# NthPortal/reservoir

Measured on AMD Instinct MI355X. Metric: elements sampled/sec (Gelem/s) + % HBM roofline, 1B Long keys k=1024, 1/2/4/8 GPU, higher is better.
Workload: dtype int64

## Files before the change

### reservoir_amd/csrc/rsv_elements.hip

```cpp
#include <algorithm>

#include "rsv_device.h"
#include "rsv_internal.h"
#include "rsv_scan.h"

namespace rsv {

namespace {

constexpr int kBlock = 256;

constexpr int kK1Unroll = 2;

constexpr unsigned kK1Grid = 256 * 20;

constexpr int kK1Win = 12;
struct K1Lds {
    uint64_t q[kBlock / 64][k1q_cap<kK1Win>()];
    uint64_t cq[kBlock / 64][kQueue];
};

__global__ __launch_bounds__(kBlock) void k1_last_writer(DrawKey dk, uint32_t k, uint64_t lo,
                                                         uint64_t hi, uint64_t g_begin,
                                                         uint64_t n_groups,
                                                         unsigned long long* __restrict__ win, K1Launch P) {
    __shared__ K1Lds L;
    const int w = threadIdx.x >> 6;
    if (P.flags & kK1Fast) k1_body_q<kK1Win, true, kBlock>(dk, k, lo, hi, g_begin, n_groups, win, L.q[w], L.cq[w], P);
    else k1_body_q<kK1Win, false, kBlock>(dk, k, lo, hi, g_begin, n_groups, win, L.q[w], L.cq[w], P);
}

template <typename Take, typename Empty, typename Keep>
__device__ __forceinline__ void slot_rule(int64_t j, unsigned long long wi, int64_t base, int64_t n, int fresh,
                                          Take&& take, Empty&& empty, Keep&& keep) {
    if (wi) take((int64_t)wi - base, (int64_t)wi, true);
    else if (j >= base && j < base + n) take(j - base, j, false);
    else if (fresh) empty((int64_t)-1);
    else keep();
}

template <typename KeyT, int R, bool kAgentWin>
__device__ __forceinline__ void resolve_registers_first(const KeyT* __restrict__ keys, int64_t base, int64_t n,
                                                        uint32_t k, unsigned long long* __restrict__ win,
                                                        KeyT* __restrict__ slot_key, int64_t* __restrict__ slot_idx,
                                                        int fresh, int64_t m, KeyT* dst, uint32_t* flag, uint32_t gen) {
    unsigned long long wi[R];
    KeyT v[R];
#pragma unroll
    for (int r = 0; r < R; ++r) {
        const uint32_t j = threadIdx.x + r * kBlock;
        if (j >= k) wi[r] = 0ull;
        else if (kAgentWin) wi[r] = __hip_atomic_load(&win[j], __ATOMIC_RELAXED, __HIP_MEMORY_SCOPE_AGENT);
        else wi[r] = win[j];
    }
#pragma unroll
    for (int r = 0; r < R; ++r) {
        const int64_t j = threadIdx.x + r * kBlock;
        if (j >= k) continue;
        KeyT x;
        slot_rule(
            j, wi[r], base, n, fresh, [&](int64_t off, int64_t, bool) { x = keys[off]; }, [&](int64_t) { x = 0; },
            [&] { x = slot_key[j]; });
        v[r] = x;
    }
#pragma unroll
    for (int r = 0; r < R; ++r) {
        const int64_t j = threadIdx.x + r * kBlock;
        if (j >= k) continue;
        const KeyT x = v[r];
        slot_rule(
            j, wi[r], base, n, fresh,
            [=](int64_t, int64_t idx, bool winner) {
                slot_key[j] = x;
                slot_idx[j] = idx;
                if (winner) win[j] = 0;
            },
            [=](int64_t idx) {
                slot_key[j] = 0;
                slot_idx[j] = idx;
            },
            [] {});
        if (j < m) dst[j] = x;
    }
    publish_flag(flag, gen);
}

constexpr uint32_t kK1FusedMaxK = 8 * kBlock;

template <typename KeyT>
__global__ __launch_bounds__(kBlock) void k1_resolve_publish(DrawKey dk, uint32_t k, uint64_t lo, uint64_t hi,
                                                             uint64_t g_begin, uint64_t n_groups,
                                                             unsigned long long* __restrict__ win,
                                                             uint32_t* ticket, const KeyT* __restrict__ keys,
                                                             int64_t base, int64_t n, KeyT* __restrict__ slot_key,
                                                             int64_t* __restrict__ slot_idx, int fresh, int64_t m,
                                                             KeyT* dst, uint32_t* flag, uint32_t gen, K1Launch P) {
    __shared__ K1Lds L;
    __shared__ uint32_t last;
    const int w = threadIdx.x >> 6;
    if (P.flags & kK1Fast) k1_body_q<kK1Win, true, kBlock>(dk, k, lo, hi, g_begin, n_groups, win, L.q[w], L.cq[w], P);
    else k1_body_q<kK1Win, false, kBlock>(dk, k, lo, hi, g_begin, n_groups, win, L.q[w], L.cq[w], P);
    asm volatile("s_waitcnt vmcnt(0)" ::: "memory");
    __syncthreads();
    if (threadIdx.x == 0) {
        const uint32_t prev = __hip_atomic_fetch_add(ticket, 1u, __ATOMIC_RELAXED, __HIP_MEMORY_SCOPE_AGENT);
        last = prev == gridDim.x - 1;
        if (last) __hip_atomic_store(ticket, 0u, __ATOMIC_RELAXED, __HIP_MEMORY_SCOPE_AGENT);
    }
    __syncthreads();
    if (!last) return;
    __builtin_amdgcn_fence(__ATOMIC_ACQUIRE, "agent");
    resolve_registers_first<KeyT, kK1FusedMaxK / kBlock, true>(keys, base, n, k, win, slot_key, slot_idx, fresh, m, dst,
                                                               flag, gen);
}

template <typename KeyT, bool kPublish>
__global__ __launch_bounds__(kPublish ? 1024 : kBlock) void resolve_kernel(const KeyT* __restrict__ keys, int64_t base,
                                                                         int64_t n, uint32_t k,
                                                                         unsigned long long* __restrict__ win,
                                                                         KeyT* __restrict__ slot_key,
                                                                         int64_t* __restrict__ slot_idx, int fresh,
                                                                         int64_t m, KeyT* dst, uint32_t* flag,
                                                                         uint32_t gen) {
    const uint32_t stride = gridDim.x * blockDim.x;
    for (uint32_t j = blockIdx.x * blockDim.x + threadIdx.x; j < k; j += stride) {
        KeyT v = 0;
        slot_rule(
            j, win[j], base, n, fresh,
            [&](int64_t off, int64_t idx, bool winner) {
                slot_key[j] = v = keys[off];
                if (kPublish || slot_idx) slot_idx[j] = idx;
                if (winner) win[j] = 0;
            },
            [=](int64_t idx) {
                slot_key[j] = 0;
                if (kPublish || slot_idx) slot_idx[j] = idx;
            },
            [&] {
                if (kPublish) v = slot_key[j];
            });
        if (kPublish && (int64_t)j < m) dst[j] = v;
    }
    if (kPublish) publish_flag(flag, gen);
}

template <typename KeyT, int R>
__global__ __launch_bounds__(kBlock) void resolve_publish_small_kernel(const KeyT* __restrict__ keys, int64_t base,
                                                                       int64_t n, uint32_t k,
                                                                       unsigned long long* __restrict__ win,
                                                                       KeyT* __restrict__ slot_key,
                                                                       int64_t* __restrict__ slot_idx, int fresh,
                                                                       int64_t m, KeyT* dst, uint32_t* flag, uint32_t gen) {
    resolve_registers_first<KeyT, R, false>(keys, base, n, k, win, slot_key, slot_idx, fresh, m, dst, flag, gen);
}

__global__ __launch_bounds__(kBlock) void replay_kernel(const int64_t* __restrict__ ev_pos,
                                                        const int32_t* __restrict__ ev_slot,
                                                        int64_t n_events, uint32_t k,
                                                        unsigned long long* __restrict__ win) {
    const int64_t e = (int64_t)blockIdx.x * blockDim.x + threadIdx.x;
    if (e >= n_events) return;
    const int32_t s = ev_slot[e];
    const int64_t p = ev_pos[e];
    if (s >= 0 && (uint32_t)s < k && p >= 2) atomicMax(&win[s], (unsigned long long)(p - 1));
}

__global__ __launch_bounds__(kBlock) void export_draws_kernel(DrawKey dk, uint64_t i0, int64_t n,
                                                              uint64_t* __restrict__ out) {
    const int64_t t = (int64_t)blockIdx.x * blockDim.x + threadIdx.x;
    if (t >= n) return;
    const uint64_t i = i0 + (uint64_t)t;
    const u32x4 w = level0(dk, i >> 4);
    out[t] = exact_j(dk, i, level0_byte(w, (uint32_t)(i & 15)));
}

template <typename KeyT>
struct StridedParts {
    using Key = KeyT;
    const int64_t* idx;
    const KeyT* key;
    int64_t part_len;
    __device__ int64_t index(int32_t p, uint32_t j) const { return idx[(int64_t)p * part_len + j]; }
    __device__ void take(int32_t p, uint32_t j, KeyT* slot_key) const { slot_key[j] = key[(int64_t)p * part_len + j]; }
};

template <typename KeyT>
struct PackedRows {
    using Key = KeyT;
    const int64_t* rows;
    int64_t stride;
    uint32_t k;
    __device__ int64_t index(int32_t p, uint32_t j) const { return rows[(int64_t)p * stride + j]; }
    __device__ void take(int32_t p, uint32_t j, KeyT* slot_key) const {
        slot_key[j] = (KeyT)rows[(int64_t)p * stride + k + j];
    }
};

struct StridedWideParts {
    using Key = uint32_t;
    const int64_t* idx;
    const uint32_t* key;
    int64_t part_len;
    uint32_t words;
    __device__ int64_t index(int32_t p, uint32_t j) const { return idx[(int64_t)p * part_len + j]; }
    __device__ void take(int32_t p, uint32_t j, uint32_t* slot_key) const {
        const uint32_t* src = key + ((size_t)p * part_len + j) * words;
        for (uint32_t q = 0; q < words; ++q) slot_key[(size_t)j * words + q] = src[q];
    }
};

struct PackedWideRows {
    using Key = uint32_t;
    const int64_t* rows;
    int64_t stride;
    uint32_t k, words;
    __device__ int64_t index(int32_t p, uint32_t j) const { return rows[(int64_t)p * stride + j]; }
    __device__ void take(int32_t p, uint32_t j, uint32_t* slot_key) const {
        const uint32_t* src = (const uint32_t*)(rows + (int64_t)p * stride + k) + (size_t)j * words;
        for (uint32_t q = 0; q < words; ++q) slot_key[(size_t)j * words + q] = src[q];
    }
};

template <typename Src>
__device__ __forceinline__ int32_t merge_winner(const Src& src, int32_t parts, uint32_t j, int64_t& best) {
    int32_t from = -1;
    for (int32_t p = 0; p < parts; ++p) {
        const int64_t idx = src.index(p, j);
        if (idx > best) {
            best = idx;
            from = p;
        }
    }
    return from;
}

template <typename Src, bool kPublish>
__global__ __launch_bounds__(kPublish ? 1024 : kBlock) void merge_kernel(Src src, int32_t parts, uint32_t k,
                                                                       int64_t* __restrict__ slot_idx,
                                                                       typename Src::Key* __restrict__ slot_key,
                                                                       int64_t m, typename Src::Key* dst,
                                                                       uint32_t* flag, uint32_t gen) {
    const uint32_t stride = gridDim.x * blockDim.x;
    for (uint32_t j = blockIdx.x * blockDim.x + threadIdx.x; j < k; j += stride) {
        int64_t best = slot_idx[j];
        const int32_t from = merge_winner(src, parts, j, best);
        if (from >= 0) {
            slot_idx[j] = best;
            src.take(from, j, slot_key);
        }
        if (kPublish && (int64_t)j < m) dst[j] = slot_key[j];
    }
    if (kPublish) publish_flag(flag, gen);
}

template <typename KeyT>
__global__ __launch_bounds__(kBlock) void export_packed_kernel(const int64_t* __restrict__ slot_idx,
                                                               const KeyT* __restrict__ slot_key, uint32_t k,
                                                               int64_t* __restrict__ row) {
    const uint32_t j = blockIdx.x * blockDim.x + threadIdx.x;
    if (j >= k) return;
    row[j] = slot_idx[j];
    row[k + j] = (int64_t)slot_key[j];
}

__global__ __launch_bounds__(1024) void resolve_wide_kernel(const uint32_t* __restrict__ keys, int64_t base,
                                                            int64_t n, uint32_t k, uint32_t words,
                                                            unsigned long long* __restrict__ win,
                                                            uint32_t* __restrict__ slot_key,
                                                            int64_t* __restrict__ slot_idx, int fresh, int64_t m,
                                                            uint32_t* dst, uint32_t* flag, uint32_t gen) {
    const uint32_t stride = gridDim.x * blockDim.x;
    for (uint32_t j = blockIdx.x * blockDim.x + threadIdx.x; j < k; j += stride) {
        const uint32_t* src = nullptr;
        bool write = true;
        slot_rule(
            j, win[j], base, n, fresh,
            [&](int64_t off, int64_t idx, bool winner) {
                src = keys + (size_t)off * words;
                slot_idx[j] = idx;
                if (winner) win[j] = 0;
            },
            [=](int64_t idx) { slot_idx[j] = idx; }, [&] { write = false; });
        uint32_t* o = slot_key + (size_t)j * words;
        const bool out = dst && (int64_t)j < m;
        for (uint32_t q = 0; q < words; ++q) {
            const uint32_t v = src ? src[q] : (write ? 0u : o[q]);
            if (write) o[q] = v;
            if (out) dst[(size_t)j * words + q] = v;
        }
    }
    if (dst) publish_flag(flag, gen);
}

__global__ __launch_bounds__(kBlock) void export_packed_wide_kernel(const int64_t* __restrict__ slot_idx,
                                                                    const uint32_t* __restrict__ slot_key, uint32_t k,
                                                                    uint32_t words, int64_t* __restrict__ row) {
    const uint32_t j = blockIdx.x * blockDim.x + threadIdx.x;
    if (j >= k) return;
    row[j] = slot_idx[j];
    uint32_t* o = (uint32_t*)(row + k) + (size_t)j * words;
    for (uint32_t q = 0; q < words; ++q) o[q] = slot_key[(size_t)j * words + q];
}

inline DrawKey make_key(const DrawParams& dp) {
    return DrawKey{(uint32_t)dp.seed, (uint32_t)(dp.seed >> 32), (uint32_t)dp.stream,
                   (uint32_t)(dp.stream >> 32)};
}

inline unsigned grid_for(uint64_t items, unsigned cap = ~0u) {
    uint64_t b = (items + kBlock - 1) / kBlock;
    if (b < 1) b = 1;
    return (unsigned)(b < cap ? b : cap);
}

inline unsigned k1_grid(uint64_t n_groups) {
    constexpr uint64_t per_window = (uint64_t)kK1Unroll * kBlock * kK1Win;
    if (n_groups < per_window * 768) return grid_for((n_groups + kK1Unroll - 1) / kK1Unroll, kK1Grid);
    const uint64_t m = std::max<uint64_t>(1, (n_groups + per_window * kK1Grid / 2) / (per_window * kK1Grid));
    return (unsigned)std::max<uint64_t>(1, n_groups / (per_window * m));
}

constexpr uint32_t kK1W1 = 256 * 6 * (kBlock / 64);
constexpr uint32_t kK1Rest = 5400, kK1MinA = 5;
inline unsigned k1_plan(uint32_t k, uint64_t lo, uint64_t hi, uint64_t g_begin, uint64_t n_groups, K1Launch& P) {
    const unsigned stride_grid = k1_grid(n_groups);
    P = k1_launch<kK1Win>(k, lo, hi, g_begin, n_groups, stride_grid, kBlock);
    if (P.units < kK1MinA * kK1W1 + kK1Rest) return stride_grid;
    const unsigned grid = k1_schedule(P, kK1W1, (P.units - kK1Rest) / kK1W1, 2, kBlock);
    return grid ? grid : stride_grid;
}

template <typename F>
hipError_t with_key_type(int key_width, F&& f) {
    if (key_width == 8) f(int64_t{});
    else f(int32_t{});
    return hipGetLastError();
}

inline unsigned one_group_threads(uint32_t k) {
    return std::min<unsigned>(1024, std::max<unsigned>(64, (k + 63) / 64 * 64));
}

}

hipError_t launch_k1_last_writer(const DrawParams& dp, uint32_t k, uint64_t lo, uint64_t hi,
                                 unsigned long long* batch_win, hipStream_t st) {
    if (hi <= lo) return hipSuccess;
    const uint64_t g_end = (hi + 15) >> 4;
    constexpr uint64_t kMaxGroups = 1ull << 31;
    uint64_t n_groups = 0;
    for (uint64_t g_begin = lo >> 4; g_begin < g_end; g_begin += n_groups) {
        const uint64_t g_wrap = ((g_begin >> 32) + 1) << 32;
        n_groups = std::min<uint64_t>(std::min<uint64_t>(g_end, g_wrap) - g_begin, kMaxGroups);
        K1Launch P;
        const unsigned grid = k1_plan(k, lo, hi, g_begin, n_groups, P);
        hipLaunchKernelGGL(k1_last_writer, dim3(grid), dim3(kBlock), 0, st, make_key(dp), k, lo, hi,
                           g_begin, n_groups, batch_win, P);
        hipError_t e = hipGetLastError();
        if (e != hipSuccess) return e;
    }
    return hipSuccess;
}

bool k1_fused_ok(uint64_t lo, uint64_t hi, uint32_t k, int key_width) {
    if (hi <= lo || k > kK1FusedMaxK || (key_width != 8 && key_width != 4)) return false;
    const uint64_t g_begin = lo >> 4, g_end = (hi + 15) >> 4;
    return g_end - g_begin <= (1ull << 31) && g_end <= ((g_begin >> 32) + 1) << 32;
}

hipError_t launch_k1_resolve_publish(const DrawParams& dp, uint64_t lo, uint64_t hi, const SlotBlock& sb,
                                     uint32_t* ticket, const Batch& b, const Publication& pub, hipStream_t st) {
    if (!k1_fused_ok(lo, hi, sb.k, sb.key_width)) return hipErrorInvalidValue;
    const uint64_t g_begin = lo >> 4, n_groups = ((hi + 15) >> 4) - g_begin;
    K1Launch P;
    const unsigned grid = k1_plan(sb.k, lo, hi, g_begin, n_groups, P);
    return with_key_type(sb.key_width, [&](auto t) {
        using T = decltype(t);
        hipLaunchKernelGGL(k1_resolve_publish<T>, dim3(grid), dim3(kBlock), 0, st, make_key(dp), sb.k, lo, hi, g_begin,
                           n_groups, sb.win, ticket, (const T*)b.keys, b.base, b.n, (T*)sb.slot_key, sb.slot_idx,
                           (int)b.fresh, pub.m, (T*)pub.dst, pub.flag, pub.gen, P);
    });
}

hipError_t launch_resolve(const SlotBlock& sb, const Batch& b, const Publication& pub, hipStream_t st, bool small) {
    const uint32_t k = sb.k;
    if (sb.key_width > 8) {
        const unsigned grid = pub.dst ? 1 : grid_for(k, 256 * 64);
        hipLaunchKernelGGL(resolve_wide_kernel, dim3(grid), dim3(pub.dst ? one_group_threads(k) : kBlock), 0, st,
                           (const uint32_t*)b.keys, b.base, b.n, k, (uint32_t)sb.key_width / 4, sb.win,
                           (uint32_t*)sb.slot_key, sb.slot_idx, (int)b.fresh, pub.m, (uint32_t*)pub.dst, pub.flag,
                           pub.gen);
        return hipGetLastError();
    }
    return with_key_type(sb.key_width, [&](auto t) {
        using T = decltype(t);
        auto go = [&](auto kernel, unsigned grid, unsigned threads) {
            hipLaunchKernelGGL(kernel, dim3(grid), dim3(threads), 0, st, (const T*)b.keys, b.base, b.n, k, sb.win,
                               (T*)sb.slot_key, sb.slot_idx, (int)b.fresh, pub.m, (T*)pub.dst, pub.flag, pub.gen);
        };
        if (!pub.dst) go(resolve_kernel<T, false>, grid_for(k), kBlock);
        else if (!(small && k <= 8 * kBlock)) go(resolve_kernel<T, true>, 1, one_group_threads(k));
        else if (k <= 2 * kBlock) go(resolve_publish_small_kernel<T, 2>, 1, kBlock);
        else if (k <= 4 * kBlock) go(resolve_publish_small_kernel<T, 4>, 1, kBlock);
        else go(resolve_publish_small_kernel<T, 8>, 1, kBlock);
    });
}

__global__ __launch_bounds__(kBlock) void init_slots_kernel(uint8_t* slot_key, int key_width, int64_t* slot_idx,
                                                            unsigned long long* win, uint32_t k, uint32_t* ticket) {
    const uint64_t stride = (uint64_t)gridDim.x * blockDim.x;
    if (ticket && blockIdx.x == 0 && threadIdx.x == 0) *ticket = 0;
    for (uint64_t j = (uint64_t)blockIdx.x * blockDim.x + threadIdx.x; j < k; j += stride) {
        win[j] = 0;
        slot_idx[j] = -1;
        if (key_width == 8)
            ((int64_t*)slot_key)[j] = 0;
        else if (key_width == 4)
            ((int32_t*)slot_key)[j] = 0;
        else
            for (int q = 0; q < key_width / 4; ++q) ((uint32_t*)slot_key)[(size_t)j * (key_width / 4) + q] = 0;
    }
}

hipError_t launch_init_slots(const SlotBlock& sb, hipStream_t st, uint32_t* ticket) {
    hipLaunchKernelGGL(init_slots_kernel, dim3(grid_for(sb.k, 256 * 64)), dim3(kBlock), 0, st, (uint8_t*)sb.slot_key,
                       sb.key_width, sb.slot_idx, sb.win, sb.k, ticket);
    return hipGetLastError();
}

__global__ __launch_bounds__(1024) void publish_kernel(const uint32_t* __restrict__ src, uint32_t* dst,
                                                      int64_t words, uint32_t* flag, uint32_t gen) {
    const int64_t vecs = words >> 2;
    for (int64_t i = threadIdx.x; i < vecs; i += blockDim.x)
        ((uint4*)dst)[i] = ((const uint4*)src)[i];
    for (int64_t i = (vecs << 2) + threadIdx.x; i < words; i += blockDim.x) dst[i] = src[i];
    publish_flag(flag, gen);
}

__global__ __launch_bounds__(1024) void publish_multi_kernel(const uint32_t* __restrict__ src, uint32_t* dst,
                                                            int64_t words, uint32_t* flag, uint32_t gen,
                                                            uint32_t* ticket) {
    const int64_t vecs = words >> 2;
    const int64_t stride = (int64_t)gridDim.x * blockDim.x;
    const int64_t t0 = (int64_t)blockIdx.x * blockDim.x + threadIdx.x;
    for (int64_t i = t0; i < vecs; i += stride) ((uint4*)dst)[i] = ((const uint4*)src)[i];
    for (int64_t i = (vecs << 2) + t0; i < words; i += stride) dst[i] = src[i];
    asm volatile("s_waitcnt vmcnt(0)" ::: "memory");
    __syncthreads();
    if (threadIdx.x == 0) {
        __threadfence_system();
        const uint32_t prev = __hip_atomic_fetch_add(ticket, 1u, __ATOMIC_ACQ_REL, __HIP_MEMORY_SCOPE_AGENT);
        if (prev == gridDim.x - 1) {
            __hip_atomic_store(ticket, 0u, __ATOMIC_RELAXED, __HIP_MEMORY_SCOPE_AGENT);
            __threadfence_system();
            __hip_atomic_store(flag, gen, __ATOMIC_RELEASE, __HIP_MEMORY_SCOPE_SYSTEM);
        }
    }
}

hipError_t launch_publish_multi(const void* src, int64_t bytes, void* dst_host_dev, uint32_t* flag_dev, uint32_t gen,
                                uint32_t* ticket_dev, hipStream_t st) {
    const int64_t per = 32 * 1024;
    const unsigned grid = (unsigned)std::min<int64_t>(32, std::max<int64_t>(1, (bytes + per - 1) / per));
    hipLaunchKernelGGL(publish_multi_kernel, dim3(grid), dim3(1024), 0, st, (const uint32_t*)src,
                       (uint32_t*)dst_host_dev, bytes / 4, flag_dev, gen, ticket_dev);
    return hipGetLastError();
}

hipError_t launch_publish(const void* src, int64_t bytes, void* dst_host_dev, uint32_t* flag_dev, uint32_t gen,
                          hipStream_t st) {
    hipLaunchKernelGGL(publish_kernel, dim3(1), dim3(1024), 0, st, (const uint32_t*)src, (uint32_t*)dst_host_dev,
                       bytes / 4, flag_dev, gen);
    return hipGetLastError();
}

__device__ __forceinline__ int64_t resolve_index_slot(uint64_t j, int64_t base, int64_t n, unsigned long long* win,
                                                      int64_t* slot_idx, int fresh, uint8_t* slot_key, int key_width) {
    int64_t off = -1;
    slot_rule(
        (int64_t)j, win[j], base, n, fresh,
        [&](int64_t o, int64_t idx, bool winner) {
            slot_idx[j] = idx;
            if (winner) win[j] = 0;
            off = o;
        },
        [=](int64_t idx) {
            slot_idx[j] = idx;
            for (int q = 0; q < key_width; ++q) slot_key[j * key_width + q] = 0;
        },
        [] {});
    return off;
}

__global__ __launch_bounds__(kBlock) void resolve_indices_kernel(int64_t base, int64_t n, uint32_t k,
                                                                 unsigned long long* __restrict__ win,
                                                                 int64_t* __restrict__ slot_idx, int fresh,
                                                                 uint8_t* __restrict__ slot_key, int key_width,
                                                                 int64_t* __restrict__ offs) {
    const uint64_t stride = (uint64_t)gridDim.x * blockDim.x;
    for (uint64_t j = (uint64_t)blockIdx.x * blockDim.x + threadIdx.x; j < k; j += stride)
        offs[j] = resolve_index_slot(j, base, n, win, slot_idx, fresh, slot_key, key_width);
}

__global__ __launch_bounds__(kBlock) void fill_slots_kernel(const int64_t* __restrict__ offs, const uint8_t* __restrict__ keys,
                                                            uint32_t k, int key_width, uint8_t* __restrict__ slot_key) {
    const uint64_t stride = (uint64_t)gridDim.x * blockDim.x;
    for (uint64_t j = (uint64_t)blockIdx.x * blockDim.x + threadIdx.x; j < k; j += stride) {
        if (offs[j] < 0) continue;
        if (key_width == 8) ((int64_t*)slot_key)[j] = ((const int64_t*)keys)[j];
        else if (key_width == 4) ((int32_t*)slot_key)[j] = ((const int32_t*)keys)[j];
        else
            for (int q = 0; q < key_width; ++q) slot_key[j * key_width + q] = keys[j * key_width + q];
    }
}


constexpr uint32_t kIdxPublishMaxK = 8192;

__global__ __launch_bounds__(1024) void resolve_indices_publish_kernel(int64_t base, int64_t n, uint32_t k,
                                                                       unsigned long long* __restrict__ win,
                                                                       int64_t* __restrict__ slot_idx, int fresh,
                                                                       uint8_t* __restrict__ slot_key, int key_width,
                                                                       int64_t* __restrict__ offs, int64_t* offs_host,
                                                                       uint32_t* flag, uint32_t gen) {
    for (uint32_t j = threadIdx.x; j < k; j += blockDim.x) {
        const int64_t off = resolve_index_slot(j, base, n, win, slot_idx, fresh, slot_key, key_width);
        offs[j] = off;
        offs_host[j] = off;
    }
    publish_flag(flag, gen);
}

template <typename KeyT>
__global__ __launch_bounds__(1024) void fill_slots_publish_kernel(const int64_t* __restrict__ offs,
                                                                  const KeyT* __restrict__ keys, uint32_t k,
                                                                  KeyT* __restrict__ slot_key, int64_t m, KeyT* dst,
                                                                  uint32_t* flag, uint32_t gen) {
    for (uint32_t j = threadIdx.x; j < k; j += blockDim.x) {
        KeyT v;
        if (offs[j] >= 0) {
            v = keys[j];
            slot_key[j] = v;
        } else {
            v = slot_key[j];
        }
        if ((int64_t)j < m) dst[j] = v;
    }
    publish_flag(flag, gen);
}

bool resolve_indices_publish_ok(uint32_t k) { return k <= kIdxPublishMaxK; }

hipError_t launch_resolve_indices(const SlotBlock& sb, const Batch& b, int64_t* offs, const Publication& pub,
                                  hipStream_t st) {
    if (!pub.dst)
        hipLaunchKernelGGL(resolve_indices_kernel, dim3(grid_for(sb.k, 256 * 64)), dim3(kBlock), 0, st, b.base, b.n, sb.k,
                           sb.win, sb.slot_idx, (int)b.fresh, (uint8_t*)sb.slot_key, sb.key_width, offs);
    else if (!resolve_indices_publish_ok(sb.k))
        return hipErrorInvalidValue;
    else
        hipLaunchKernelGGL(resolve_indices_publish_kernel, dim3(1), dim3(one_group_threads(sb.k)), 0, st, b.base, b.n,
                           sb.k, sb.win, sb.slot_idx, (int)b.fresh, (uint8_t*)sb.slot_key, sb.key_width, offs,
                           (int64_t*)pub.dst, pub.flag, pub.gen);
    return hipGetLastError();
}

bool fill_slots_publish_ok(uint32_t k, int key_width) {
    return k <= kIdxPublishMaxK && (key_width == 4 || key_width == 8);
}

hipError_t launch_fill_slots(const int64_t* offs, const void* keys, const SlotBlock& sb, const Publication& pub,
                             hipStream_t st) {
    if (!pub.dst) {
        hipLaunchKernelGGL(fill_slots_kernel, dim3(grid_for(sb.k, 256 * 64)), dim3(kBlock), 0, st, offs,
                           (const uint8_t*)keys, sb.k, sb.key_width, (uint8_t*)sb.slot_key);
        return hipGetLastError();
    }
    if (!fill_slots_publish_ok(sb.k, sb.key_width)) return hipErrorInvalidValue;
    return with_key_type(sb.key_width, [&](auto t) {
        using T = decltype(t);
        hipLaunchKernelGGL(fill_slots_publish_kernel<T>, dim3(1), dim3(one_group_threads(sb.k)), 0, st, offs,
                           (const T*)keys, sb.k, (T*)sb.slot_key, pub.m, (T*)pub.dst, pub.flag, pub.gen);
    });
}

hipError_t launch_replay_events(const int64_t* ev_pos, const int32_t* ev_slot, int64_t n_events,
                                uint32_t k, unsigned long long* batch_win, hipStream_t st) {
    if (n_events <= 0) return hipSuccess;
    const unsigned grid = (unsigned)((n_events + kBlock - 1) / kBlock);
    hipLaunchKernelGGL(replay_kernel, dim3(grid), dim3(kBlock), 0, st, ev_pos, ev_slot, n_events, k,
                       batch_win);
    return hipGetLastError();
}

hipError_t launch_export_draws(const DrawParams& dp, uint64_t i0, int64_t n, uint64_t* j,
                               hipStream_t st) {
    if (n <= 0) return hipSuccess;
    const unsigned grid = (unsigned)((n + kBlock - 1) / kBlock);
    hipLaunchKernelGGL(export_draws_kernel, dim3(grid), dim3(kBlock), 0, st, make_key(dp), i0, n, j);
    return hipGetLastError();
}

namespace {

template <bool kPublish, typename Src>
void launch_merge(const Src& src, int32_t parts, const SlotBlock& sb, const Publication& pub, hipStream_t st) {
    using Key = typename Src::Key;
    hipLaunchKernelGGL((merge_kernel<Src, kPublish>), dim3(kPublish ? 1 : grid_for(sb.k)),
                       dim3(kPublish ? one_group_threads(sb.k) : kBlock), 0, st, src, parts, sb.k, sb.slot_idx,
                       (Key*)sb.slot_key, pub.m, (Key*)pub.dst, pub.flag, pub.gen);
}

}

hipError_t launch_merge_slots(const int64_t* idx_parts, const void* key_parts, int32_t parts, int64_t part_len,
                              const SlotBlock& sb, hipStream_t st) {
    if (sb.key_width > 8) {
        const StridedWideParts src{idx_parts, (const uint32_t*)key_parts, part_len, (uint32_t)sb.key_width / 4};
        launch_merge<false>(src, parts, sb, Publication{}, st);
        return hipGetLastError();
    }
    return with_key_type(sb.key_width, [&](auto t) {
        using T = decltype(t);
        launch_merge<false>(StridedParts<T>{idx_parts, (const T*)key_parts, part_len}, parts, sb, Publication{}, st);
    });
}

hipError_t launch_export_packed(const SlotBlock& sb, int64_t* row, hipStream_t st) {
    if (sb.key_width > 8) {
        hipLaunchKernelGGL(export_packed_wide_kernel, dim3(grid_for(sb.k)), dim3(kBlock), 0, st, sb.slot_idx,
                           (const uint32_t*)sb.slot_key, sb.k, (uint32_t)sb.key_width / 4, row);
        return hipGetLastError();
    }
    return with_key_type(sb.key_width, [&](auto t) {
        using T = decltype(t);
        hipLaunchKernelGGL(export_packed_kernel<T>, dim3(grid_for(sb.k)), dim3(kBlock), 0, st, sb.slot_idx,
                           (const T*)sb.slot_key, sb.k, row);
    });
}

hipError_t launch_merge_packed(const int64_t* rows, int32_t parts, int64_t stride, const SlotBlock& sb,
                               const Publication& pub, hipStream_t st) {
    if (sb.key_width > 8) {
        if (pub.dst) return hipErrorInvalidValue;
        launch_merge<false>(PackedWideRows{rows, stride, sb.k, (uint32_t)sb.key_width / 4}, parts, sb, pub, st);
        return hipGetLastError();
    }
    return with_key_type(sb.key_width, [&](auto t) {
        using T = decltype(t);
        const PackedRows<T> src{rows, stride, sb.k};
        if (pub.dst) launch_merge<true>(src, parts, sb, pub, st);
        else launch_merge<false>(src, parts, sb, pub, st);
    });
}

}
```

### reservoir_amd/csrc/rsv_scan.h

```cpp
#pragma once
#include <algorithm>

#include "rsv_device.h"

namespace rsv {

constexpr uint32_t kQueue = 128;
constexpr uint64_t kIndexMask = (1ull << 56) - 1;

__device__ __forceinline__ uint32_t clip_mask16(uint64_t i0, uint64_t lo, uint64_t hi) {
    uint32_t m = 0xFFFFu;
    if (i0 < lo) m = (lo - i0 >= 16) ? 0u : ((0xFFFFu << (uint32_t)(lo - i0)) & 0xFFFFu);
    if (i0 + 16 > hi) m &= (hi <= i0) ? 0u : (0xFFFFu >> (uint32_t)(16 - (hi - i0)));
    return m;
}

__device__ __forceinline__ uint32_t candidate_mask16(const u32x4& w, uint64_t i0, uint64_t dense_lim) {
    if (i0 + 1 >= dense_lim) return zero_byte_mask16(w);
    const float Tf = __fdividef((float)dense_lim, (float)(i0 + 1));
    if (Tf > 300.0f) return 0xFFFFu;
    uint32_t T = (uint32_t)Tf;
    if ((uint64_t)T * (i0 + 1) < dense_lim) ++T;
    if (T > 0 && (uint64_t)(T - 1) * (i0 + 1) >= dense_lim) --T;
    return lt_mask16(w, T > 256u ? 256u : T);
}

template <class Hit>
__device__ __forceinline__ void resolve_entry(const DrawKey& dk, uint64_t e, uint32_t k, Hit& hit) {
    const uint64_t i = e & kIndexMask;
    const uint64_t j = exact_j(dk, i, (uint32_t)(e >> 56));
    if (j < k) hit((uint32_t)j, i);
}

template <class Hit>
__device__ __forceinline__ void enqueue_block(const DrawKey& dk, const u32x4& w, uint64_t i0,
                                              uint32_t mask, uint64_t* q, uint32_t& qn,
                                              uint32_t lane, uint32_t k, Hit& hit) {
    while (__any(mask != 0)) {
        const bool has = mask != 0;
        const unsigned long long bal = __ballot(has);
        if (has) {
            const uint32_t e = __builtin_ctz(mask);
            mask &= mask - 1;
            const uint32_t pos = __builtin_amdgcn_mbcnt_hi((uint32_t)(bal >> 32), __builtin_amdgcn_mbcnt_lo((uint32_t)bal, 0u));
            q[qn + pos] = ((uint64_t)level0_byte(w, e) << 56) | (i0 + e);
        }
        qn += (uint32_t)__popcll(bal);
        if (qn >= 64) {
            qn -= 64;
            __builtin_amdgcn_wave_barrier();
            resolve_entry(dk, q[qn + lane], k, hit);
            __builtin_amdgcn_wave_barrier();
        }
    }
}

template <class Hit>
__device__ __forceinline__ void drain_queue(const DrawKey& dk, const uint64_t* q, uint32_t& qn,
                                            uint32_t lane, uint32_t k, Hit& hit) {
    __builtin_amdgcn_wave_barrier();
    if (lane < qn) resolve_entry(dk, q[lane], k, hit);
    qn = 0;
    __builtin_amdgcn_wave_barrier();
}


template <class Hit>
__device__ __forceinline__ void resolve_block(const DrawKey& dk, bool valid, uint64_t g, uint64_t lo,
                                              uint64_t hi, uint64_t dense_lim, uint32_t k, uint64_t* cq,
                                              uint32_t& cqn, uint32_t lane, Hit& hit) {
    const u32x4 w = level0(dk, g);
    const uint64_t i0 = g << 4;
    uint32_t mask = valid ? candidate_mask16(w, i0, dense_lim) : 0u;
    if (i0 < lo || i0 + 16 > hi) mask &= clip_mask16(i0, lo, hi);
    if (mask) {
        const uint32_t e = __builtin_ctz(mask);
        mask &= mask - 1;
        const uint64_t j = exact_j(dk, i0 + e, level0_byte(w, e));
        if (j < k) hit((uint32_t)j, i0 + e);
    }
    enqueue_block(dk, w, i0, mask, cq, cqn, lane, k, hit);
}

__device__ __forceinline__ uint32_t fold16(const u32x4& w) {
    const uint32_t x = w.x | w.y | w.z | w.w;
    uint32_t y;
    asm("v_or_b32_sdwa %0, %1, %1 dst_sel:WORD_0 dst_unused:UNUSED_PAD src0_sel:WORD_0 src1_sel:WORD_1\n\t"
        "s_nop 0"
        : "=v"(y)
        : "v"(x));
    return y;
}

__device__ __forceinline__ u32x4 level1_b0_words(const DrawKey& dk, uint64_t i, bool hi_uniform, uint32_t c1u) {
    const uint64_t g1 = i >> 1;
    if (hi_uniform) return philox4x32_10_uniform_hi((uint32_t)g1, c1u, dk.s0, dk.s1, dk.k0, dk.k1);
    return philox4x32_10((uint32_t)g1, (uint32_t)(g1 >> 32) | kDomainLevel1, dk.s0, dk.s1, dk.k0, dk.k1);
}

__device__ __forceinline__ uint32_t fold_pair(const u32x4& a, const u32x4& b) {
    const uint32_t xa = a.x | a.y | a.z | a.w, xb = b.x | b.y | b.z | b.w;
    uint32_t z;
    asm("v_or_b32_sdwa %0, %1, %1 dst_sel:WORD_0 dst_unused:UNUSED_PAD src0_sel:WORD_0 src1_sel:WORD_1\n\t"
        "s_nop 0\n\t"
        "v_or_b32_sdwa %0, %2, %2 dst_sel:WORD_1 dst_unused:UNUSED_PRESERVE src0_sel:WORD_0 src1_sel:WORD_1\n\t"
        "s_nop 0"
        : "=&v"(z)
        : "v"(xa), "v"(xb));
    return z;
}

template <int W>
constexpr uint32_t k1q_cap() { return 64u * (1u + W / 2); }
constexpr uint32_t kQueueWaves = 4;


constexpr uint32_t kK1Fast = 1u, kK1HiUniform = 2u, kK1Below2p40 = 4u;
struct K1Launch {
    uint32_t W1, A, B;
    uint32_t nB;
    uint32_t units;
    uint32_t unit_off;
    uint32_t head_iters;
    uint32_t slow_iters;
    uint32_t tail_off;
    uint32_t stride;
    uint32_t off_steady, ng_steady;
    uint32_t c1u, ghi;
    uint32_t flags;
    uint64_t k24, khi;
};

template <int W = 12>
inline K1Launch k1_launch(uint32_t k, uint64_t lo, uint64_t hi, uint64_t g_begin, uint64_t n_groups, unsigned grid,
                          unsigned block = 256) {
    constexpr uint32_t UB = (W / 2) * 2 * 64, IB = 2 * 64;
    K1Launch P{};
    const uint32_t ng = (uint32_t)n_groups;
    const uint64_t g_sparse = (256ull * k + 14) >> 4;
    const uint32_t off_sparse = g_sparse <= g_begin ? 0u : (uint32_t)std::min<uint64_t>(g_sparse - g_begin, ng);
    P.off_steady = std::max<uint32_t>(off_sparse, (lo & 15) ? 1u : 0u);
    P.ng_steady = ng - ((hi & 15) ? 1u : 0u);
    P.stride = grid * block * 2;
    P.c1u = (uint32_t)(lo >> 33) | kDomainLevel1;
    P.ghi = (uint32_t)(g_begin >> 32);
    const bool hi_uniform = (lo >> 33) == ((hi - 1) >> 33), below = hi <= (1ull << 40);
    P.flags = (hi_uniform && below ? kK1Fast : 0u) | (hi_uniform ? kK1HiUniform : 0u) | (below ? kK1Below2p40 : 0u);
    P.k24 = (uint64_t)k << 24;
    P.khi = (uint64_t)k << 32;
    const uint32_t head = (uint32_t)std::min<uint64_t>(((uint64_t)P.off_steady + IB - 1) / IB * IB, ng);
    P.unit_off = head;
    P.units = P.ng_steady > head ? (P.ng_steady - head) / UB : 0u;
    P.tail_off = head + P.units * UB;
    P.head_iters = (head + IB - 1) / IB;
    P.slow_iters = P.head_iters + (ng - P.tail_off + IB - 1) / IB;
    return P;
}

inline unsigned k1_schedule(K1Launch& P, uint32_t W1, uint32_t A, uint32_t B, unsigned block = 256) {
    if (W1 == 0 || A == 0 || B == 0 || (uint64_t)W1 * A >= P.units) return 0;
    const uint64_t rest = P.units - (uint64_t)W1 * A;
    const uint64_t wpg = block / 64, waves = W1 + (rest + B - 1) / B;
    const unsigned grid = (unsigned)((waves + wpg - 1) / wpg);
    P.W1 = W1;
    P.A = A;
    P.B = B;
    P.nB = (uint32_t)(grid * wpg - W1);
    P.stride = grid * block * 2;
    return grid;
}

template <int W = 12, bool FAST = false, int BS = 256>
__device__ __forceinline__ void k1_body_q(const DrawKey& dk, uint32_t k, uint64_t lo, uint64_t hi, uint64_t g_begin,
                                          uint64_t n_groups, unsigned long long* __restrict__ win, uint64_t* q,
                                          uint64_t* cq, const K1Launch& P, uint32_t* pool = nullptr) {
    static_assert(W % 2 == 0, "half windows");
    constexpr int U = 2;
    const uint32_t lane = threadIdx.x & 63;
    uint32_t qn = 0, cqn = 0;
    auto hit = [&](uint32_t j, uint64_t i) { atomicMax(&win[j], (unsigned long long)i); };
    const uint64_t dense_lim = 256ull * k;
    const uint32_t ng = (uint32_t)n_groups;
    const uint32_t stride = P.stride;
    const uint32_t c1u = P.c1u;
    const bool hi_uniform = P.flags & kK1HiUniform;
    const bool pre_ok = P.flags & kK1Below2p40;
    const uint64_t k_hi = P.khi, k_24 = P.k24;
    int32_t dpend = 0;
    const uint32_t g0 = (uint32_t)g_begin;
    uint32_t base = __builtin_amdgcn_readfirstlane((blockIdx.x * BS + (threadIdx.x & ~63u)) * U);
    const uint32_t ghi = P.ghi;
    uint32_t gl = g0 + base + lane;
    const uint32_t off_steady = P.off_steady, ng_steady = P.ng_steady;

    auto resolve = [&](bool valid, uint64_t ent) {
        const uint32_t gt = (uint32_t)ent * kPhiloxM0Inv, off = gt - g0, z = (uint32_t)(ent >> 32);
        __builtin_assume(!valid || z != 0xFFFFFFFFu);
        bool dense = false;
        if (dpend > 0) {
            dense = valid && ((z & 0xFFFFu) == 0 || (z >> 16) == 0);
            const unsigned long long db = __builtin_amdgcn_ballot_w64(dense);
            if (db) {
                resolve_block(dk, dense, g_begin + off, lo, hi, dense_lim, k, cq, cqn, lane, hit);
                resolve_block(dk, dense && off + 64 < ng, g_begin + off + 64, lo, hi, dense_lim, k, cq, cqn, lane, hit);
                dpend -= std::min<int32_t>(dpend, (int32_t)__popcll(db));
            }
        }
        const uint32_t zm = (valid && !dense) ? ~z : 0u;
        uint32_t rest = 0;
        if (zm) {
            const uint32_t e = __builtin_ctz(zm);
            rest = zm & (zm - 1);
            if constexpr (FAST) {
                const uint32_t bl = gt + ((e & 16u) << 2);
                const uint32_t g1lo = (bl << 3) | ((e & 15u) >> 1);
                const u32x4 w = philox4x32_10_uniform_hi(g1lo, c1u, dk.s0, dk.s1, dk.k0, dk.k1);
                const bool odd = e & 1u;
                const uint32_t Lh = odd ? w.z : w.x;
                const uint32_t i8 = (ghi << 28) | (bl >> 4);
                if ((uint64_t)(Lh >> 8) * i8 < k_24) {
                    const uint64_t i = ((((uint64_t)ghi << 32) | bl) << 4) | (e & 15u);
                    const uint64_t L = ((uint64_t)Lh << 32) | (odd ? w.w : w.y);
                    const uint64_t j = __umul64hi(L >> 8, i + 1);
                    if (j < k) hit((uint32_t)j, i);
                }
            } else {
                const uint64_t i = ((g_begin + off + ((e >> 4) << 6)) << 4) + (e & 15u);
                const u32x4 w = level1_b0_words(dk, i, hi_uniform, c1u);
                const uint32_t Lh = (i & 1) ? w.z : w.x;
                const bool maybe = !pre_ok || (uint64_t)(Lh >> 8) * (i + 1) < k_hi;
                if (maybe) {
                    const uint64_t L = ((uint64_t)Lh << 32) | ((i & 1) ? w.w : w.y);
                    const uint64_t j = __umul64hi(L >> 8, i + 1);
                    if (j < k) hit((uint32_t)j, i);
                }
            }
        }
        const unsigned long long bal = __builtin_amdgcn_ballot_w64(rest != 0);
        if (bal) {
            if (rest) {
                const uint32_t pos = __builtin_amdgcn_mbcnt_hi((uint32_t)(bal >> 32), __builtin_amdgcn_mbcnt_lo((uint32_t)bal, 0u));
                q[qn + pos] = (uint64_t)(uint32_t)ent | ((uint64_t)~rest << 32);
            }
            qn += (uint32_t)__popcll(bal);
        }
    };
    auto rounds = [&]() {
        while (qn >= 64) {
            qn -= 64;
            __builtin_amdgcn_wave_barrier();
            const uint64_t ent = q[qn + lane];
            __builtin_amdgcn_wave_barrier();
            resolve(true, ent);
            __builtin_amdgcn_wave_barrier();
        }
    };
    auto append = [&](bool has, uint32_t gt, uint32_t z) {
        const unsigned long long bal = __builtin_amdgcn_ballot_w64(has);
        if (has) {
            const uint32_t pos = __builtin_amdgcn_mbcnt_hi((uint32_t)(bal >> 32), __builtin_amdgcn_mbcnt_lo((uint32_t)bal, 0u));
            q[qn + pos] = (uint64_t)gt | ((uint64_t)z << 32);
        }
        qn += (uint32_t)__popcll(bal);
    };

    const uint32_t q_s = (uint32_t)__builtin_amdgcn_readfirstlane((int)(uint32_t)(uintptr_t)q);
    uint32_t m0v;
    asm volatile("v_mov_b32 %0, %1" : "=v"(m0v) : "s"(kPhiloxM0));
    auto steady = [&](uint32_t d) {
        u32x4 w0, w1;
        uint32_t glo;
        philox4x32_10_uniform_hi_x2_at(gl, m0v, (uint64_t)kPhiloxM0 * d, ghi, dk.s0, dk.s1, dk.k0, dk.k1, w0, w1, glo);
        const uint32_t xa = w0.x | w0.y | w0.z | w0.w, xb = w1.x | w1.y | w1.z | w1.w;
        uint32_t z;
        unsigned long long m;
        asm("v_or_b32_sdwa %0, %2, %2 dst_sel:WORD_0 dst_unused:UNUSED_PAD src0_sel:WORD_0 src1_sel:WORD_1\n\t"
            "s_nop 0\n\t"
            "v_or_b32_sdwa %0, %3, %3 dst_sel:WORD_1 dst_unused:UNUSED_PRESERVE src0_sel:WORD_0 src1_sel:WORD_1\n\t"
            "s_nop 0\n\t"
            "v_cmp_ne_u32_e64 %1, -1, %0"
            : "=&v"(z), "=s"(m)
            : "v"(xa), "v"(xb));
        const uint32_t pos = __builtin_amdgcn_mbcnt_hi((uint32_t)(m >> 32), __builtin_amdgcn_mbcnt_lo((uint32_t)m, 0u));
        const uint32_t sb = q_s + 8u * qn;
        const uint64_t ent = (uint64_t)glo | ((uint64_t)z << 32);
        unsigned long long sv;
        uint32_t addr;
        asm volatile("v_lshl_add_u32 %1, %2, 3, %3\n\t"
                     "s_mov_b64 %0, exec\n\t"
                     "s_mov_b64 exec, %4\n\t"
                     "ds_write_b64 %1, %5\n\t"
                     "s_mov_b64 exec, %0"
                     : "=&s"(sv), "=&v"(addr)
                     : "v"(pos), "s"(sb), "s"(m), "v"(ent)
                     : "memory");
        qn += (uint32_t)__popcll(m);
    };
    auto partial = [&](uint32_t b) {
        u32x4 w[U];
#pragma unroll
        for (int u = 0; u < U; ++u)
            w[u] = philox4x32_10_uniform_hi(gl, ghi, dk.s0, dk.s1, dk.k0, dk.k1, (uint64_t)kPhiloxM0 * (64u * u));
        uint32_t z;
        bool has;
        if (b >= off_steady && b + U * 64 <= ng_steady) {
            z = fold_pair(w[0], w[1]);
            has = z != 0xFFFFFFFFu;
        } else {
            uint32_t y[U];
            bool hb[U];
#pragma unroll
            for (int u = 0; u < U; ++u) {
                const uint32_t off = b + u * 64 + lane;
                const uint64_t i0 = (g_begin + off) << 4;
                const bool dense = i0 + 1 < dense_lim;
                y[u] = off >= ng ? 0xFFFFu
                                 : dense ? 0u : (fold16(w[u]) | (~clip_mask16(i0, lo, hi) & 0xFFFFu));
                hb[u] = (off < ng) & (dense | ((uint16_t)y[u] != 0xFFFFu));
            }
            z = (y[0] & 0xFFFFu) | (y[1] << 16);
            has = hb[0] | hb[1];
        }
        dpend += (int32_t)__popcll(__builtin_amdgcn_ballot_w64(has && ((z & 0xFFFFu) == 0 || (z >> 16) == 0)));
        append(has, gl * kPhiloxM0, z);
        __builtin_amdgcn_wave_barrier();
        rounds();
    };
    if (P.A > 0) {
        constexpr uint32_t UB = (W / 2) * U * 64;
        const uint32_t W1 = P.W1;
        const uint32_t wg = __builtin_amdgcn_readfirstlane((blockIdx.x * BS + threadIdx.x) >> 6);
        const bool ga = wg < W1;
        if (ga) {
            for (uint32_t d = wg; d < P.slow_iters; d += W1) {
                const uint32_t b = d < P.head_iters ? d * (U * 64) : P.tail_off + (d - P.head_iters) * (U * 64);
                gl = g0 + b + lane;
                partial(b);
            }
        }
        const uint32_t cnt = ga ? P.A : P.B, u_step = ga ? W1 : P.nB, u_first = ga ? wg : W1 * P.A + (wg - W1);
        for (uint32_t j = 0; j < cnt; ++j) {
            const uint32_t u = u_first + j * u_step;
            if (u >= P.units) break;
            gl = g0 + P.unit_off + u * UB + lane;
#pragma unroll
            for (int t = 0; t < W / 2; ++t) steady(t * (U * 64));
            __builtin_amdgcn_wave_barrier();
            rounds();
        }
        base = ng;
    }
    while (base < ng) {
        if (base >= off_steady && (uint64_t)base + (uint64_t)(W - 1) * stride + U * 64 <= ng_steady) {
#pragma unroll
            for (int h = 0; h < 2; ++h) {
#pragma unroll
                for (int t = 0; t < W / 2; ++t) steady(t * stride);
                gl += (W / 2) * stride;
                __builtin_amdgcn_wave_barrier();
                rounds();
            }
            base += W * stride;
        } else {
            for (int t = 0; t < W && base < ng; ++t, base += stride, gl += stride) {
                partial(base);
            }
        }
    }
    if (pool) {
        constexpr uint32_t cap = k1q_cap<W>(), NW = kQueueWaves;
        const uint32_t wv = threadIdx.x >> 6;
        const uint64_t* q0 = q - (size_t)wv * cap;
        for (;;) {
            if (lane == 0) pool[wv] = qn | (dpend > 0 ? 0x80000000u : 0u);
            __syncthreads();
            uint32_t c[NW], T = 0, anyd = 0;
#pragma unroll
            for (uint32_t v = 0; v < NW; ++v) {
                const uint32_t pv = (uint32_t)__builtin_amdgcn_readfirstlane((int)pool[v]);
                c[v] = pv & 0x7FFFFFFFu;
                anyd |= pv >> 31;
                T += c[v];
            }
            if (T == 0) break;
            uint32_t o = 64u * wv + lane, src = 0;
            const bool valid = o < T;
#pragma unroll
            for (uint32_t v = 0; v + 1 < NW; ++v)
                if (src == v && o >= c[v]) {
                    o -= c[v];
                    src = v + 1;
                }
            const uint64_t ent = valid ? q0[(size_t)src * cap + o] : 0ull;
            __syncthreads();
            qn = 0;
            dpend = anyd ? (1 << 30) : 0;
            if (64u * wv < T) resolve(valid, ent);
        }
    } else {
        while (qn > 0) {
            __builtin_amdgcn_wave_barrier();
            const uint32_t nv = std::min<uint32_t>(qn, 64u);
            qn -= nv;
            const bool valid = lane < nv;
            const uint64_t ent = valid ? q[qn + lane] : 0ull;
            __builtin_amdgcn_wave_barrier();
            resolve(valid, ent);
        }
    }
    __builtin_amdgcn_wave_barrier();
    drain_queue(dk, cq, cqn, lane, k, hit);
}

}
```

Baseline: 11600.

## Use LDS atomic queue top with deferred writes and template fast path

Adds a per-wave LDS 'top' counter and a pipelined steady path. Each half-window step reserves queue slots with ds_add_rtn_u32 and writes the previous step's entry in the next step, so the write overlaps the next Philox compute instead of depending on a scalar prefix position. The FAST flag becomes a template parameter chosen on the host, which removes the runtime branch and leaves one body instantiation per kernel. The resolve-publish tail arguments are packed into a struct that is read through the kernarg pointer after the scan, to cut register and SGPR pressure during the hot loop. Risks are the extra LDS atomics and added waitcnt stalls, and the qn bookkeeping now has to stay consistent with the atomic top.

```diff
diff --git a/reservoir_amd/csrc/rsv_elements.hip b/reservoir_amd/csrc/rsv_elements.hip
--- a/reservoir_amd/csrc/rsv_elements.hip
+++ b/reservoir_amd/csrc/rsv_elements.hip
@@ -18,16 +18,18 @@
 struct K1Lds {
     uint64_t q[kBlock / 64][k1q_cap<kK1Win>()];
     uint64_t cq[kBlock / 64][kQueue];
+    uint32_t top[kBlock / 64];
 };
 
+template <bool FAST>
 __global__ __launch_bounds__(kBlock) void k1_last_writer(DrawKey dk, uint32_t k, uint64_t lo,
                                                          uint64_t hi, uint64_t g_begin,
                                                          uint64_t n_groups,
                                                          unsigned long long* __restrict__ win, K1Launch P) {
     __shared__ K1Lds L;
     const int w = threadIdx.x >> 6;
-    if (P.flags & kK1Fast) k1_body_q<kK1Win, true, kBlock>(dk, k, lo, hi, g_begin, n_groups, win, L.q[w], L.cq[w], P);
-    else k1_body_q<kK1Win, false, kBlock>(dk, k, lo, hi, g_begin, n_groups, win, L.q[w], L.cq[w], P);
+    k1_body_q<kK1Win, FAST, kBlock, true>(dk, k, lo, hi, g_begin, n_groups, win, L.q[w], L.cq[w], P, nullptr,
+                                          &L.top[w]);
 }
 
 template <typename Take, typename Empty, typename Keep>
@@ -88,30 +90,48 @@
 constexpr uint32_t kK1FusedMaxK = 8 * kBlock;
 
 template <typename KeyT>
-__global__ __launch_bounds__(kBlock) void k1_resolve_publish(DrawKey dk, uint32_t k, uint64_t lo, uint64_t hi,
-                                                             uint64_t g_begin, uint64_t n_groups,
-                                                             unsigned long long* __restrict__ win,
-                                                             uint32_t* ticket, const KeyT* __restrict__ keys,
-                                                             int64_t base, int64_t n, KeyT* __restrict__ slot_key,
-                                                             int64_t* __restrict__ slot_idx, int fresh, int64_t m,
-                                                             KeyT* dst, uint32_t* flag, uint32_t gen, K1Launch P) {
+struct K1Tail {
+    uint32_t* ticket;
+    const KeyT* keys;
+    int64_t base, n;
+    KeyT* slot_key;
+    int64_t* slot_idx;
+    int64_t m;
+    KeyT* dst;
+    uint32_t* flag;
+    uint32_t gen;
+    int fresh;
+    uint32_t grid;
+};
+
+template <typename KeyT, bool FAST>
+__global__ __launch_bounds__(kBlock) void k1_resolve_publish(K1Tail<KeyT>, DrawKey dk, uint32_t k, uint64_t lo,
+                                                             uint64_t hi, uint64_t g_begin, uint64_t n_groups,
+                                                             unsigned long long* __restrict__ win, K1Launch P) {
     __shared__ K1Lds L;
     __shared__ uint32_t last;
+    __shared__ uint64_t tail_at;
     const int w = threadIdx.x >> 6;
-    if (P.flags & kK1Fast) k1_body_q<kK1Win, true, kBlock>(dk, k, lo, hi, g_begin, n_groups, win, L.q[w], L.cq[w], P);
-    else k1_body_q<kK1Win, false, kBlock>(dk, k, lo, hi, g_begin, n_groups, win, L.q[w], L.cq[w], P);
+    tail_at = (uint64_t)__builtin_amdgcn_kernarg_segment_ptr();
+    k1_body_q<kK1Win, FAST, kBlock, true>(dk, k, lo, hi, g_begin, n_groups, win, L.q[w], L.cq[w], P, nullptr,
+                                          &L.top[w]);
+    asm volatile("" ::: "memory");
+    const uint64_t at = tail_at;
+    const uint64_t args = ((uint64_t)(uint32_t)__builtin_amdgcn_readfirstlane((int)(at >> 32)) << 32) |
+                          (uint32_t)__builtin_amdgcn_readfirstlane((int)at);
+    const auto* T = (const __attribute__((address_space(4))) K1Tail<KeyT>*)args;
     asm volatile("s_waitcnt vmcnt(0)" ::: "memory");
     __syncthreads();
     if (threadIdx.x == 0) {
-        const uint32_t prev = __hip_atomic_fetch_add(ticket, 1u, __ATOMIC_RELAXED, __HIP_MEMORY_SCOPE_AGENT);
-        last = prev == gridDim.x - 1;
-        if (last) __hip_atomic_store(ticket, 0u, __ATOMIC_RELAXED, __HIP_MEMORY_SCOPE_AGENT);
+        const uint32_t prev = __hip_atomic_fetch_add(T->ticket, 1u, __ATOMIC_RELAXED, __HIP_MEMORY_SCOPE_AGENT);
+        last = prev == T->grid - 1;
+        if (last) __hip_atomic_store(T->ticket, 0u, __ATOMIC_RELAXED, __HIP_MEMORY_SCOPE_AGENT);
     }
     __syncthreads();
     if (!last) return;
     __builtin_amdgcn_fence(__ATOMIC_ACQUIRE, "agent");
-    resolve_registers_first<KeyT, kK1FusedMaxK / kBlock, true>(keys, base, n, k, win, slot_key, slot_idx, fresh, m, dst,
-                                                               flag, gen);
+    resolve_registers_first<KeyT, kK1FusedMaxK / kBlock, true>(T->keys, T->base, T->n, k, win, T->slot_key, T->slot_idx,
+                                                               T->fresh, T->m, T->dst, T->flag, T->gen);
 }
 
 template <typename KeyT, bool kPublish>
@@ -330,6 +350,12 @@
     return grid ? grid : stride_grid;
 }
 
+inline auto k1_last_writer_for(const K1Launch& P) { return k1_fast_form(P) ? k1_last_writer<true> : k1_last_writer<false>; }
+template <typename KeyT>
+inline auto k1_resolve_publish_for(const K1Launch& P) {
+    return k1_fast_form(P) ? k1_resolve_publish<KeyT, true> : k1_resolve_publish<KeyT, false>;
+}
+
 template <typename F>
 hipError_t with_key_type(int key_width, F&& f) {
     if (key_width == 8) f(int64_t{});
@@ -354,8 +380,9 @@
         n_groups = std::min<uint64_t>(std::min<uint64_t>(g_end, g_wrap) - g_begin, kMaxGroups);
         K1Launch P;
         const unsigned grid = k1_plan(k, lo, hi, g_begin, n_groups, P);
-        hipLaunchKernelGGL(k1_last_writer, dim3(grid), dim3(kBlock), 0, st, make_key(dp), k, lo, hi,
-                           g_begin, n_groups, batch_win, P);
+        const auto kernel = k1_last_writer_for(P);
+        hipLaunchKernelGGL(kernel, dim3(grid), dim3(kBlock), 0, st, make_key(dp), k, lo, hi, g_begin, n_groups,
+                           batch_win, P);
         hipError_t e = hipGetLastError();
         if (e != hipSuccess) return e;
     }
@@ -376,9 +403,11 @@
     const unsigned grid = k1_plan(sb.k, lo, hi, g_begin, n_groups, P);
     return with_key_type(sb.key_width, [&](auto t) {
         using T = decltype(t);
-        hipLaunchKernelGGL(k1_resolve_publish<T>, dim3(grid), dim3(kBlock), 0, st, make_key(dp), sb.k, lo, hi, g_begin,
-                           n_groups, sb.win, ticket, (const T*)b.keys, b.base, b.n, (T*)sb.slot_key, sb.slot_idx,
-                           (int)b.fresh, pub.m, (T*)pub.dst, pub.flag, pub.gen, P);
+        const auto kernel = k1_resolve_publish_for<T>(P);
+        const K1Tail<T> tail{ticket, (const T*)b.keys, b.base, b.n,  (T*)sb.slot_key, sb.slot_idx,
+                             pub.m,  (T*)pub.dst,      pub.flag, pub.gen, (int)b.fresh, grid};
+        hipLaunchKernelGGL(kernel, dim3(grid), dim3(kBlock), 0, st, tail, make_key(dp), sb.k, lo, hi, g_begin, n_groups,
+                           sb.win, P);
     });
 }
 
diff --git a/reservoir_amd/csrc/rsv_scan.h b/reservoir_amd/csrc/rsv_scan.h
--- a/reservoir_amd/csrc/rsv_scan.h
+++ b/reservoir_amd/csrc/rsv_scan.h
@@ -1,5 +1,6 @@
 #pragma once
 #include <algorithm>
+#include <type_traits>
 
 #include "rsv_device.h"
 
@@ -157,6 +158,8 @@
     return P;
 }
 
+inline bool k1_fast_form(const K1Launch& P) { return (P.flags & kK1Fast) != 0; }
+
 inline unsigned k1_schedule(K1Launch& P, uint32_t W1, uint32_t A, uint32_t B, unsigned block = 256) {
     if (W1 == 0 || A == 0 || B == 0 || (uint64_t)W1 * A >= P.units) return 0;
     const uint64_t rest = P.units - (uint64_t)W1 * A;
@@ -170,10 +173,11 @@
     return grid;
 }
 
-template <int W = 12, bool FAST = false, int BS = 256>
+template <int W = 12, bool FAST = false, int BS = 256, bool TOP = false>
 __device__ __forceinline__ void k1_body_q(const DrawKey& dk, uint32_t k, uint64_t lo, uint64_t hi, uint64_t g_begin,
                                           uint64_t n_groups, unsigned long long* __restrict__ win, uint64_t* q,
-                                          uint64_t* cq, const K1Launch& P, uint32_t* pool = nullptr) {
+                                          uint64_t* cq, const K1Launch& P, uint32_t* pool = nullptr,
+                                          uint32_t* top = nullptr) {
     static_assert(W % 2 == 0, "half windows");
     constexpr int U = 2;
     const uint32_t lane = threadIdx.x & 63;
@@ -296,6 +300,85 @@
                      : "memory");
         qn += (uint32_t)__popcll(m);
     };
+    struct Pending {
+        uint32_t glo, z, addr;
+        unsigned long long m;
+    };
+    uint32_t top_v = 0, eight_v = 0;
+    if constexpr (TOP) {
+        const uint32_t top_s = (uint32_t)__builtin_amdgcn_readfirstlane((int)(uint32_t)(uintptr_t)top);
+        asm volatile("v_mov_b32 %0, %1" : "=v"(top_v) : "s"(top_s));
+        asm volatile("v_mov_b32 %0, 8" : "=v"(eight_v));
+    }
+    auto top_set = [&]() {
+        uint32_t t;
+        asm volatile("v_mov_b32 %0, %2\n\t"
+                     "ds_write_b32 %1, %0"
+                     : "=&v"(t)
+                     : "v"(top_v), "s"(q_s + 8u * qn)
+                     : "memory");
+    };
+    auto steady_top = [&](uint32_t d, const Pending& prev, auto first) -> Pending {
+        u32x4 w0, w1;
+        Pending cur;
+        philox4x32_10_uniform_hi_x2_at(gl, m0v, (uint64_t)kPhiloxM0 * d, ghi, dk.s0, dk.s1, dk.k0, dk.k1, w0, w1, cur.glo);
+        const uint32_t xa = w0.x | w0.y | w0.z | w0.w, xb = w1.x | w1.y | w1.z | w1.w;
+        asm("v_or_b32_sdwa %0, %2, %2 dst_sel:WORD_0 dst_unused:UNUSED_PAD src0_sel:WORD_0 src1_sel:WORD_1\n\t"
+            "s_nop 0\n\t"
+            "v_or_b32_sdwa %0, %3, %3 dst_sel:WORD_1 dst_unused:UNUSED_PRESERVE src0_sel:WORD_0 src1_sel:WORD_1\n\t"
+            "s_nop 0\n\t"
+            "v_cmp_ne_u32_e64 %1, -1, %0"
+            : "=&v"(cur.z), "=s"(cur.m)
+            : "v"(xa), "v"(xb));
+        unsigned long long sv;
+        if constexpr (decltype(first)::value) {
+            asm volatile("s_mov_b64 %0, exec\n\t"
+                         "s_mov_b64 exec, %2\n\t"
+                         "ds_add_rtn_u32 %1, %3, %4\n\t"
+                         "s_mov_b64 exec, %0"
+                         : "=&s"(sv), "=&v"(cur.addr)
+                         : "s"(cur.m), "v"(top_v), "v"(eight_v)
+                         : "memory");
+        } else {
+            const uint64_t ent = (uint64_t)prev.glo | ((uint64_t)prev.z << 32);
+            asm volatile("s_waitcnt lgkmcnt(0)\n\t"
+                         "s_mov_b64 %0, exec\n\t"
+                         "s_mov_b64 exec, %5\n\t"
+                         "ds_write_b64 %6, %7\n\t"
+                         "s_mov_b64 exec, %2\n\t"
+                         "ds_add_rtn_u32 %1, %3, %4\n\t"
+                         "s_mov_b64 exec, %0"
+                         : "=&s"(sv), "=&v"(cur.addr)
+                         : "s"(cur.m), "v"(top_v), "v"(eight_v), "s"(prev.m), "v"(prev.addr), "v"(ent)
+                         : "memory");
+        }
+        qn += (uint32_t)__popcll(cur.m);
+        return cur;
+    };
+    auto put_last = [&](const Pending& prev) {
+        const uint64_t ent = (uint64_t)prev.glo | ((uint64_t)prev.z << 32);
+        unsigned long long sv;
+        asm volatile("s_waitcnt lgkmcnt(0)\n\t"
+                     "s_mov_b64 %0, exec\n\t"
+                     "s_mov_b64 exec, %1\n\t"
+                     "ds_write_b64 %2, %3\n\t"
+                     "s_mov_b64 exec, %0"
+                     : "=&s"(sv)
+                     : "s"(prev.m), "v"(prev.addr), "v"(ent)
+                     : "memory");
+    };
+    auto half_window = [&](uint32_t step) {
+        if constexpr (TOP) {
+            top_set();
+            Pending p = steady_top(0, Pending{}, std::true_type{});
+#pragma unroll
+            for (int t = 1; t < W / 2; ++t) p = steady_top(t * step, p, std::false_type{});
+            put_last(p);
+        } else {
+#pragma unroll
+            for (int t = 0; t < W / 2; ++t) steady(t * step);
+        }
+    };
     auto partial = [&](uint32_t b) {
         u32x4 w[U];
 #pragma unroll
@@ -343,8 +426,7 @@
             const uint32_t u = u_first + j * u_step;
             if (u >= P.units) break;
             gl = g0 + P.unit_off + u * UB + lane;
-#pragma unroll
-            for (int t = 0; t < W / 2; ++t) steady(t * (U * 64));
+            half_window(U * 64);
             __builtin_amdgcn_wave_barrier();
             rounds();
         }
@@ -354,8 +436,7 @@
         if (base >= off_steady && (uint64_t)base + (uint64_t)(W - 1) * stride + U * 64 <= ng_steady) {
 #pragma unroll
             for (int h = 0; h < 2; ++h) {
-#pragma unroll
-                for (int t = 0; t < W / 2; ++t) steady(t * stride);
+                half_window(stride);
                 gl += (W / 2) * stride;
                 __builtin_amdgcn_wave_barrier();
                 rounds();
```

After: 12150 (median of 6 runs). 1.05x the previous value.
